# sirandreww/citizensassemblies-replication

Hardware: AMD Instinct MI355X
Metric: LEGACY panels/sec (node) at sf_e_110 shape; XtX MFMA util; speedup vs CPU (higher is better)
Workload: dtype int32/u64 (integer draw), fp4 MFMA -> exact int pairs; 1 GPU; sf_e_110: 1000000 LEGACY panels/GPU/step, k=110, n=1727, C=7, F=31, counts+pairs+unique; instance=sf_e_110, parallelism=panel shards x1, pipeline=draws on their own stream, 2 steps ahead of the counting

## Files before the change

### citizensassemblies-replication_amd/_native.py

```python
import ctypes
import os
import subprocess

HERE = os.path.dirname(os.path.abspath(__file__))
REPO = os.path.dirname(HERE)
LIB_PATH = os.environ.get("CSA_LIB") or os.path.join(HERE, "libcsa_legacy.so")
SRC = os.path.join(HERE, "csrc", "csa_legacy.hip")
SRC_MT = os.path.join(HERE, "csrc", "legacy_mt.cpp")
HEADER = os.path.join(REPO, "include", "csa_legacy.h")

CSA_OK = 0
CSA_E_INVALID = 1
CSA_E_BAD_QUOTAS = 2
CSA_E_NO_CANDIDATE = 3
CSA_E_ATTEMPT_LIMIT = 4
CSA_E_UNSUPPORTED = 5
CSA_E_HIP = 6
CSA_E_SELECTION = 7

CSA_WANT_PANELS = 0x1
CSA_WANT_COUNTS = 0x2
CSA_WANT_PAIRS = 0x4
CSA_WANT_UNIQUE = 0x8

CSA_PAIR_FP4 = 0
CSA_PAIR_I8 = 1
CSA_PAIR_OVERWRITE = 0x100
CSA_PAIR_SHARED = 0x200
CSA_PAIR_ALONE = 0x400
CSA_DRAW_RESET_STATUS = 0x1
CSA_DRAW_RESET_STATS = 0x2
CSA_PORTFOLIO_ACCUMULATE = 0x1
CSA_GROUP_WHIST_ACCUMULATE = 0x1
CSA_PRICE_ACCUMULATE = 0x1
CSA_PRICE_NONE = 0xFFFFFFFFFFFFFFFF
CSA_ADDRESS_GENERAL = 0
CSA_ADDRESS_BATCH = 1
CSA_MAXIMIN_START = 0x1
CSA_NASH_START = 0x1

_P = ctypes.c_void_p
_I32 = ctypes.c_int32
_U32 = ctypes.c_uint32
_U64 = ctypes.c_uint64
SIGNATURES = {
    "csa_version": (ctypes.c_int, []),
    "csa_last_error": (ctypes.c_char_p, []),
    "csa_device_count": (ctypes.c_int, [_P]),
    "csa_current_device": (ctypes.c_int, [_P]),
    "csa_instance_create": (ctypes.c_int, [_I32, _I32, _I32, _P, _P, _P, _P, _P]),
    "csa_instance_destroy": (None, [_P]),
    "csa_instance_info": (ctypes.c_int, [_P, _P, _P, _P, _P]),
    "csa_instance_set_state": (ctypes.c_int, [_P, _P, _P, _P]),
    "csa_legacy_sample": (ctypes.c_int, [_P, _I32, _U64, _U64, _U64, _U32, _U32, _P, _P, _P, _P, _P]),
    "csa_legacy_sample_devices": (ctypes.c_int, [_P, _P, _I32, _I32, _U64, _U64, _U64, _U32, _U32, _P, _P, _P,
                                                 _P, _P]),
    "csa_legacy_find": (ctypes.c_int, [_P, _I32, _U64, _U64, _U64, _U32, _P, _P]),
    "csa_legacy_attempt": (ctypes.c_int, [_P, _I32, _U64, _U64, _U32, _P, _P, _P, _P, _P]),
    "csa_first_panel_not_in": (ctypes.c_int, [_P, _I32, _U64, _U64, _U64, _U32, _P, _U64, _U64, _P, _P]),
    "csa_draw_round_panels": (ctypes.c_int, [_P, _I32, _P]),
    "csa_draw_async": (ctypes.c_int, [_P, _I32, _U64, _U64, _U64, _U32, _P, _P, _P, _P, _P, _P]),
    "csa_redraw_async": (ctypes.c_int, [_P, _I32, _U64, _U64, _U64, _U32, _P, _P, _P]),
    "csa_picks_stride": (_I32, [_I32]),
    "csa_draw_picks_supported": (ctypes.c_int, [_P, _I32]),
    "csa_draw_picks_async": (ctypes.c_int, [_P, _I32, _U64, _U64, _U64, _U32, _P, _P, _P, _P]),
    "csa_picks_pack_async": (ctypes.c_int, [_P, _U64, _I32, _I32, _P, _P, _P]),
    "csa_panel_hash_async": (ctypes.c_int, [_P, _U64, _I32, _P, _P]),
    "csa_draw_kernel_name": (ctypes.c_int, [_P, _I32, ctypes.c_char_p, _U64]),
    "csa_draw_kernel_list": (ctypes.c_int, [ctypes.c_char_p, _U64]),
    "csa_xt_pad": (_I32, [_I32]),
    "csa_transpose_count_async": (ctypes.c_int, [_P, _U64, _I32, _P, _P, _P]),
    "csa_pair_scratch_bytes": (_U64, [_I32, _U64, _U32]),
    "csa_pair_counts_ex_async": (ctypes.c_int, [_P, _U64, _I32, _P, _U32, _P, _U64, _P]),
    "csa_pair_counts_async": (ctypes.c_int, [_P, _U64, _I32, _P, _P]),
    "csa_unique_async": (ctypes.c_int, [_P, _P, _U64, _I32, _P, _U64, _P, _P, _P]),
    "csa_unique_mult_scratch_bytes": (_U64, [_U64]),
    "csa_unique_mult_async": (ctypes.c_int, [_P, _P, _U64, _I32, _P, _U64, _P, _P, _P, _P, _P]),
    "csa_mult_spectrum_async": (ctypes.c_int, [_P, _P, _U64, _P, _U64, _P, _P]),
    "csa_pair_histogram_async": (ctypes.c_int, [_P, _I32, _P, _U64, _P, _P]),
    "csa_unique_segments_async": (ctypes.c_int, [_P, _P, _U32, _U64, _P, _I32, _P, _U64, _P, _P, _P]),
    "csa_exchange_scratch_bytes": (_U64, [_U64]),
    "csa_exchange_pack_async": (ctypes.c_int, [_P, _P, _U64, _I32, _U32, _U64, _P, _U64, _P, _P, _P, _P, _P]),
    "csa_pairs_pack_async": (ctypes.c_int, [_P, _I32, _P, _P]),
    "csa_pairs_unpack_async": (ctypes.c_int, [_P, _I32, _P, _P]),
    "csa_pairs_upper_async": (ctypes.c_int, [_P, _I32, ctypes.c_double, _P, _P]),
    "csa_pairs_diag_async": (ctypes.c_int, [_P, _I32, _P, _P]),
    "csa_portfolio_pairs_async": (ctypes.c_int, [_P, _U64, _I32, _P, _P, _P, _U32, _P]),
    "csa_group_hist_async": (ctypes.c_int, [_P, _U64, _I32, _P, _I32, _I32, _P, _P, _P]),
    "csa_group_whist_scratch_bytes": (_U64, [_U64, _I32]),
    "csa_group_whist_scratch": (ctypes.c_int, [_P, _U64]),
    "csa_group_whist_async": (ctypes.c_int, [_P, _U64, _I32, _P, _P, _I32, _I32, _P, _U32, _P, _P]),
    "csa_draw_xt_async": (ctypes.c_int, [_P, _I32, _U64, _U64, _U64, _U32, _P, _P, _P, _P, _P, _P, _U32, _P]),
    "csa_status_decode": (ctypes.c_int, [_P]),
    "csa_legacy_draw_mt": (ctypes.c_int, [_I32, _I32, _I32, _P, _P, _P, _P, _P, _P, _P, _I32, _P, _U64, _U32,
                                          _I32, _P, _P, _P, _P, _P, _P, _P]),
    "csa_instance_set_address": (ctypes.c_int, [_P, _P]),
    "csa_instance_set_address_route": (ctypes.c_int, [_P, _I32]),
    "csa_draw_household_kernel_list": (ctypes.c_int, [ctypes.c_char_p, _U64]),
    "csa_instance_draw_stats": (ctypes.c_int, [_P, _I32, _P]),
    "csa_instance_draw_stats_reset": (ctypes.c_int, [_P, _P]),
    "csa_instance_draw_stats_async": (ctypes.c_int, [_P, _P, _P]),
    "csa_exchange_keys_async": (ctypes.c_int, [_P, _P, _U64, _I32, _U64, _U32, _U64, _P, _U64, _P, _P, _P, _P]),
    "csa_unique_keys_scratch_bytes": (_U64, [_U64, _I32]),
    "csa_unique_keys_async": (ctypes.c_int, [_P, _I32, _U64, _U32, _P, _U32, _U64, _P, _P, _U64, _P, _P, _P]),
    "csa_exchange_mult_keys_async": (ctypes.c_int, [_P, _U64, _P, _P, _P, _U64, _U32, _U64, _P, _P, _P, _P]),
    "csa_merge_mult_keys_scratch_bytes": (_U64, [_U64, _I32]),
    "csa_merge_mult_keys_async": (ctypes.c_int, [_P, _I32, _U64, _U32, _P, _U32, _U64, _P, _P, _U64, _P, _P, _P, _P,
                                                 _P]),
    "csa_rows_sort_tile": (_I32, []),
    "csa_rows_sort_scratch_bytes": (_U64, [_U64, _I32]),
    "csa_rows_sort_unique_async": (ctypes.c_int, [_P, _U64, _I32, _U64, _P, _U64, _P, _P, _P, _P, _P, _P]),
    "csa_rows_merge_scratch_bytes": (_U64, [_U64, _U64, _I32]),
    "csa_rows_merge_unique_async": (ctypes.c_int, [_P, _P, _P, _P, _U64, _P, _P, _P, _P, _U64, _I32, _P, _U64, _P, _P,
                                                   _P, _U64, _P, _P, _P]),
    "csa_rows_join_scratch_bytes": (_U64, [_U64, _U64, _I32]),
    "csa_rows_join_async": (ctypes.c_int, [_P, _P, _P, _U64, _P, _P, _P, _U64, _I32, _U32, _U64, _U64, _P, _U64, _P,
                                           _P, _P, _U64, _P, _P, _P, _P]),
    "csa_rows_find_async": (ctypes.c_int, [_P, _P, _U64, _I32, _P, _U64, _P, _P]),
    "csa_rows_price_tile": (_U64, []),
    "csa_rows_price_scratch_bytes": (_U64, [_U64, _I32]),
    "csa_rows_price_async": (ctypes.c_int, [_P, _P, _U64, _I32, _I32, _P, _U64, _U32, _P, _P, _P, _U64, _P]),
    "csa_rows_mw_cover_async": (ctypes.c_int, [_P, _P, _U64, _I32, _I32, _U32, _P, _P, _P, _P, _P, _U64, _P]),
    "csa_rows_first_holder_async": (ctypes.c_int, [_P, _P, _U64, _I32, _I32, _P, _P]),
    "csa_rows_maximin_scratch_bytes": (_U64, [_U64, _I32]),
    "csa_rows_maximin_async": (ctypes.c_int, [_P, _P, _U64, _I32, _I32, _U32, ctypes.c_double, _U32, _U32, _P, _P, _P,
# ... 94 lines not shown
```

### citizensassemblies-replication_amd/csrc/csa_legacy.hip

```cpp
#include <hip/hip_runtime.h>

#include <algorithm>
#include <type_traits>
#include <cstdlib>
#include <cstdarg>
#include <cstdio>
#include <cstring>
#include <string>
#include <vector>

#include "../../include/csa_legacy.h"

namespace {

thread_local std::string g_err;

int fail(int code, const char *fmt, ...) {
    char buf[512];
    va_list ap;
    va_start(ap, fmt);
    vsnprintf(buf, sizeof buf, fmt, ap);
    va_end(ap);
    g_err = buf;
    return code;
// ... 626 lines not shown
        }
    }
    __syncthreads();
    for (int p = threadIdx.x; p < np; p += blockDim.x)
        if (cnt[p]) atomicAdd(reinterpret_cast<unsigned long long *>(counts + p0 + p), (unsigned long long)cnt[p]);
}

typedef int v4i __attribute__((ext_vector_type(4)));
typedef int v8i __attribute__((ext_vector_type(8)));
typedef int v16i __attribute__((ext_vector_type(16)));
typedef float v16f __attribute__((ext_vector_type(16)));

constexpr int kPairBlock = 256;
constexpr int kPairThreads = 512;
constexpr int kPairKB = 8;

__device__ __forceinline__ v4i i8_frag(uint64_t w, int ks, int h) {
    const uint32_t x = (uint32_t)(w >> (32 * ks));
    v4i r;
#pragma unroll
    for (int q = 0; q < 4; ++q) r[q] = (int)((x >> (4 * h + q)) & 0x01010101u);
    return r;
}

__device__ __forceinline__ v8i f4_frag_a(uint32_t x) {
    v8i r;
    r[0] = (int)(x & 0x11111111u);
    r[1] = (int)(x & 0x22222222u);
    r[2] = (int)(x & 0x44444444u);
    r[3] = (int)((x >> 1) & 0x44444444u);
    r[4] = r[5] = r[6] = r[7] = 0;
    return r;
}
__device__ __forceinline__ v8i f4_frag_b(uint32_t x) {
    v8i r;
    r[0] = (int)((x << 2) & 0x44444444u);
    r[1] = (int)(x & 0x22222222u);
    r[2] = (int)((x >> 2) & 0x11111111u);
    r[3] = (int)((x >> 3) & 0x11111111u);
    r[4] = r[5] = r[6] = r[7] = 0;
    return r;
}

__device__ __forceinline__ void tri_block(int tri, int nbt, int &bi, int &bj) {
    bi = 0;
    int rem = tri;
    while (rem >= nbt - bi) {
        rem -= nbt - bi;
        ++bi;
    }
    bj = bi + rem;
}

template <bool FP4, bool PARTIAL, int KB>
__global__ __launch_bounds__(kPairThreads) void pair_mfma_kernel(const uint64_t *__restrict__ xt,
                                                                 uint64_t nblk, int n, int npad,
                                                                 int nbt, int nsplit,
                                                                 int64_t *__restrict__ pairs,
                                                                 int32_t *__restrict__ part) {
    __shared__ uint64_t words[2][KB][2 * kPairBlock];
    const int t = threadIdx.x, lane = t & 63, wave = t >> 6;
    const int g = (int)blockIdx.x, G = (int)gridDim.x, ntri = nbt * (nbt + 1) / 2;
    const int xcd = g & 7, it = xcd * (G >> 3) + min(xcd, G & 7) + (g >> 3);
    const int split = it / ntri, tri = it - split * ntri;
    const int item = tri * nsplit + split;
    int bi, bj;
    tri_block(tri, nbt, bi, bj);
    const int I0 = bi * kPairBlock, J0 = bj * kPairBlock;
    const uint64_t per = (nblk + nsplit - 1) / nsplit;
    const uint64_t kb0 = min(nblk, (uint64_t)split * per), kb1 = min(nblk, kb0 + per);

    using acc_t = typename std::conditional<FP4, v16f, v16i>::type;
    acc_t acc[4][2];
#pragma unroll
    for (int a = 0; a < 4; ++a)
#pragma unroll
        for (int b = 0; b < 2; ++b)
#pragma unroll
            for (int v = 0; v < 16; ++v) acc[a][b][v] = 0;

    const int wr = wave >> 2, wc = wave & 3;
    const int r32 = lane & 31, h = lane >> 5;
    const int src = t < kPairBlock ? I0 + t : J0 + t - kPairBlock;
    uint64_t nw[KB];
    const uint64_t nst = (kb1 - kb0 + KB - 1) / KB;
    auto load_stage = [&](uint64_t s) {
#pragma unroll
        for (int j = 0; j < KB; ++j) {
            const uint64_t b = kb0 + s * KB + j;
            const uint32_t *x32 = reinterpret_cast<const uint32_t *>(xt) + 2 * b * (uint64_t)npad + src;
            nw[j] = b < kb1 ? ((uint64_t)x32[0] | ((uint64_t)x32[npad] << 32)) : 0ull;
        }
    };
    if (nst) {
        load_stage(0);
#pragma unroll
        for (int j = 0; j < KB; ++j) words[0][j][t] = nw[j];
        if (nst > 1) load_stage(1);
    }
    __syncthreads();
    for (uint64_t s = 0; s < nst; ++s) {
        const int buf = (int)(s & 1);
#pragma unroll
        for (int j = 0; j < KB; ++j) {
            {
                const uint64_t *w = words[buf][j];
                if constexpr (FP4) {
                    const uint32_t *w32 = reinterpret_cast<const uint32_t *>(w) + h;
                    v8i fa[4], fb[2];
#pragma unroll
                    for (int x = 0; x < 4; ++x) fa[x] = f4_frag_a(w32[2 * (128 * wr + 32 * x + r32)]);
#pragma unroll
                    for (int x = 0; x < 2; ++x) fb[x] = f4_frag_b(w32[2 * (kPairBlock + 64 * wc + 32 * x + r32)]);
#pragma unroll
                    for (int a = 0; a < 4; ++a)
#pragma unroll
                        for (int b = 0; b < 2; ++b)
                            acc[a][b] = __builtin_amdgcn_mfma_scale_f32_32x32x64_f8f6f4(
                                fa[a], fb[b], acc[a][b], 4, 4, 0, 0x7F7F7F7F, 0, 0x7F7F7F7F);
                } else {
                    uint64_t wa[4], wb[2];
#pragma unroll
                    for (int x = 0; x < 4; ++x) wa[x] = w[128 * wr + 32 * x + r32];
#pragma unroll
                    for (int x = 0; x < 2; ++x) wb[x] = w[kPairBlock + 64 * wc + 32 * x + r32];
#pragma unroll
                    for (int ks = 0; ks < 2; ++ks) {
                        v4i fa[4], fb[2];
#pragma unroll
                        for (int x = 0; x < 4; ++x) fa[x] = i8_frag(wa[x], ks, h);
#pragma unroll
                        for (int x = 0; x < 2; ++x) fb[x] = i8_frag(wb[x], ks, h);
#pragma unroll
                        for (int a = 0; a < 4; ++a)
#pragma unroll
                            for (int b = 0; b < 2; ++b)
                                acc[a][b] = __builtin_amdgcn_mfma_i32_32x32x32_i8(fa[a], fb[b], acc[a][b], 0, 0, 0);
                    }
                }
            }
            if (j == 0) {
                if (s + 1 < nst) {
#pragma unroll
                    for (int jj = 0; jj < KB; ++jj) words[buf ^ 1][jj][t] = nw[jj];
                }
                if (s + 2 < nst) load_stage(s + 2);
            }
        }
        __syncthreads();
    }
    const int rloc = 128 * wr + 4 * h, cloc = 64 * wc + r32;
    if constexpr (PARTIAL) {
        int32_t *dst = part + (size_t)item * kPairBlock * kPairBlock;
#pragma unroll
        for (int a = 0; a < 4; ++a)
#pragma unroll
            for (int b = 0; b < 2; ++b)
#pragma unroll
                for (int v = 0; v < 16; ++v) {
                    const int row = rloc + 32 * a + (v & 3) + 8 * (v >> 2);
                    dst[row * kPairBlock + cloc + 32 * b] = (int)acc[a][b][v];
                }
    } else {
#pragma unroll
        for (int a = 0; a < 4; ++a)
#pragma unroll
            for (int b = 0; b < 2; ++b) {
                const int col = J0 + cloc + 32 * b;
#pragma unroll
                for (int v = 0; v < 16; ++v) {
                    const int row = I0 + rloc + 32 * a + (v & 3) + 8 * (v >> 2);
                    const int val = (int)acc[a][b][v];
                    if (val != 0 && row < n && col < n)
                        atomicAdd(reinterpret_cast<unsigned long long *>(pairs + (uint64_t)row * n + col),
                                  (unsigned long long)(long long)val);
                }
                __builtin_amdgcn_sched_barrier(0);
            }
    }
}

__global__ __launch_bounds__(256) void pair_reduce_kernel(const int32_t *__restrict__ part, int n, int nbt,
                                                          int nsplit, int64_t *__restrict__ pairs,
                                                          int overwrite) {
    int bi, bj;
    tri_block((int)blockIdx.y, nbt, bi, bj);
    const int e = blockIdx.x * 256 + threadIdx.x;
    const int row = bi * kPairBlock + (e >> 8), col = bj * kPairBlock + (e & 255);
    if (row >= n || col >= n) return;
    const int32_t *p = part + (size_t)blockIdx.y * nsplit * kPairBlock * kPairBlock + e;
    int64_t acc = 0;
    for (int k = 0; k < nsplit; ++k) acc += p[(size_t)k * kPairBlock * kPairBlock];
    if (overwrite) pairs[(size_t)row * n + col] = acc;
    else if (acc) pairs[(size_t)row * n + col] += acc;
}

constexpr int kP2Threads = 256;
constexpr int kP2Depth = 8;
constexpr int kP2Xcds = 8;
constexpr uint64_t kP2MaxBlocks = ((1ull << 24) - 1) / 64;

struct PairMap {
    int nbt, ntri, P;
    int halves;
    uint64_t nblk;
    __host__ __device__ int nitems() const { return ntri * halves; }
    __host__ __device__ void item_at(int idx, int &bi, int &bj, int &c0) const {
        tile_at(idx / halves, bi, bj);
        c0 = (idx % halves) * (kPairBlock / halves);
    }
    __host__ __device__ void tile_at(int idx, int &bi, int &bj) const {
        int r0 = 0;
        for (;;) {
            const int hb = nbt - r0 < 4 ? nbt - r0 : 4;
            const int cnt = hb * (hb + 1) / 2 + (nbt - r0 - hb) * hb;
            if (idx < cnt) break;
            idx -= cnt;
            r0 += 4;
        }
        const int hb = nbt - r0 < 4 ? nbt - r0 : 4;
        const int tri = hb * (hb + 1) / 2;
        if (idx < tri) {
            int c = 0;
            while (idx > c) {
                idx -= c + 1;
                ++c;
            }
            bj = r0 + c;
            bi = r0 + idx;
        } else {
            idx -= tri;
            bj = r0 + hb + idx / hb;
            bi = r0 + idx % hb;
        }
    }
    __host__ __device__ void xcd_chunk(int x, int &t0, int &tx) const {
        t0 = (int)((int64_t)nitems() * x / kP2Xcds);
        tx = (int)((int64_t)nitems() * (x + 1) / kP2Xcds) - t0;
    }
    __host__ __device__ int leftovers() const {
        int tl = 0;
        for (int x = 0; x < kP2Xcds; ++x) {
            int t0, tx;
// ... 1540 lines not shown
    for (const DrawConfig &c : kDrawKernels) {
        draw_config_name(c, name, sizeof name);
        all += name;
        all += '\n';
    }
    if (!buf || len < all.size() + 1)
        return fail(CSA_E_INVALID, "draw kernel list: the buffer needs %zu bytes", all.size() + 1);
    memcpy(buf, all.c_str(), all.size() + 1);
    return CSA_OK;
}

int csa_draw_household_kernel_list(char *buf, uint64_t len) {
    std::string all;
    char name[128];
    for (const DrawConfig &c : kHouseholdKernels) {
        draw_config_name(c, name, sizeof name);
        all += name;
        all += '\n';
    }
    if (!buf || len < all.size() + 1)
        return fail(CSA_E_INVALID, "household kernel list: the buffer needs %zu bytes", all.size() + 1);
    memcpy(buf, all.c_str(), all.size() + 1);
    return CSA_OK;
}

int32_t csa_xt_pad(int32_t n) { return ((n + kPairBlock - 1) / kPairBlock) * kPairBlock; }

int csa_transpose_count_async(const uint64_t *d_panels, uint64_t n_panels, int32_t n, uint64_t *d_xt,
                              int64_t *d_counts, void *stream) {
    if (n <= 0 || !d_panels || !d_counts) return fail(CSA_E_INVALID, "transpose: bad arguments");
    if (n_panels == 0) return CSA_OK;
    const int W = (n + 63) / 64, CW = std::min(W, kXtCols), Wp = CW | 1;
    const size_t lds = (size_t)64 * Wp * 8 + (size_t)std::min(n, 64 * CW) * 4;
    if (lds > 160 * 1024) return fail(CSA_E_UNSUPPORTED, "transpose needs %zu B of LDS", lds);
    const uint64_t nblk = (n_panels + 63) / 64;
    const unsigned ranges = (unsigned)((W + kXtCols - 1) / kXtCols);
    static int cus = 0;
    if (!cus) {
        int dev = 0;
        if (hipGetDevice(&dev) != hipSuccess ||
            hipDeviceGetAttribute(&cus, hipDeviceAttributeMultiprocessorCount, dev) != hipSuccess || cus <= 0)
            cus = 256;
    }
    const uint64_t bpg = std::max<uint64_t>(1, std::min<uint64_t>(kXtBlocksPerGroup, nblk * ranges / (2 * (uint64_t)cus)));
    const unsigned grid = (unsigned)((nblk + bpg - 1) / bpg);
    hipLaunchKernelGGL(xt_count_kernel, dim3(grid, ranges), dim3(kXtThreads), lds, (hipStream_t)stream, d_panels,
                       n_panels, n, W, csa_xt_pad(n), d_xt, d_counts, (int)bpg);
    HIPCHK(hipGetLastError());
    return CSA_OK;
}

namespace {
struct PairPlan {
    int npad, nbt, ntri, nsplit;
};

int pair_plan(int32_t n, uint64_t n_blocks, uint32_t engine, PairPlan &p) {
    if (engine != CSA_PAIR_FP4 && engine != CSA_PAIR_I8) return fail(CSA_E_INVALID, "pairs: unknown engine %u", engine);
    p.npad = csa_xt_pad(n);
    p.nbt = p.npad / kPairBlock;
    p.ntri = p.nbt * (p.nbt + 1) / 2;
    int cus = 256;
    int dev = 0;
    if (hipGetDevice(&dev) == hipSuccess) (void)hipDeviceGetAttribute(&cus, hipDeviceAttributeMultiprocessorCount, dev);
    const uint64_t ns_cap = std::max<uint64_t>(1, n_blocks / 8);
    uint64_t ns = std::max(1, cus / p.ntri);
    if (2 * p.ntri > cus) {
        auto cost = [&](uint64_t m) { return (double)((p.ntri * m + cus - 1) / cus) / (double)m; };
        const uint64_t hi = std::min<uint64_t>(64, ns_cap);
        double best = cost(1);
        for (uint64_t m = 2; m <= hi; ++m) best = std::min(best, cost(m));
        ns = 1;
        while (ns < hi && cost(ns) > 1.02 * best) ++ns;
    }
    ns = std::min<uint64_t>(ns, ns_cap);
    const uint64_t exact_blocks = engine == CSA_PAIR_FP4 ? (1ull << 24) / 64 : (1ull << 31) / 64;
    ns = std::max<uint64_t>(ns, (n_blocks + exact_blocks - 1) / exact_blocks);
    if (ns > (1u << 20)) return fail(CSA_E_UNSUPPORTED, "pairs: too many panel blocks per call");
    p.nsplit = (int)ns;
    return CSA_OK;
}
struct Pair2Plan {
    PairMap M;
    int grid = 0, lmax = 0;
};

constexpr uint64_t kP2AloneMinBlocks = 2048;
constexpr int kP2AloneMinTiles = 4;
bool pair2_plan(int32_t n, uint64_t n_blocks, uint32_t engine, bool shared, Pair2Plan &q, bool alone = false) {
    if (engine != CSA_PAIR_FP4 || n_blocks == 0 || n_blocks > kP2MaxBlocks) return false;
    const char *e = getenv("CSA_PAIR_KERNEL");
    const int force = e ? atoi(e) : 0;
    if (force == 1) return false;
    int cus = 256, dev = 0;
    if (hipGetDevice(&dev) == hipSuccess) (void)hipDeviceGetAttribute(&cus, hipDeviceAttributeMultiprocessorCount, dev);
    if (cus < kP2Xcds || cus % kP2Xcds) return false;
    (void)shared;
    const char *enb = getenv("CSA_P2_NB");
    const int nbf = enb ? atoi(enb) : 4;
    q.M.halves = nbf == 2 ? 2 : 1;
    q.M.nbt = csa_xt_pad(n) / kPairBlock;
    q.M.ntri = q.M.nbt * (q.M.nbt + 1) / 2;
    q.M.P = cus / kP2Xcds;
    q.M.nblk = n_blocks;
    q.grid = cus;
    q.lmax = q.M.leftovers();
    static const uint64_t alone_min_blocks = [] {
        const char *v = getenv("CSA_PAIR_ALONE_MIN_BLOCKS");
        return v ? (uint64_t)strtoull(v, nullptr, 10) : kP2AloneMinBlocks;
    }();
    alone = alone && n_blocks >= alone_min_blocks && q.M.nbt >= kP2AloneMinTiles;
    return force == 2 || alone || q.M.ntri >= cus;
}

uint64_t pair2_scratch_bytes(const Pair2Plan &q) {
    return q.lmax ? (uint64_t)q.lmax * q.M.pieces(q.lmax) * kPairBlock * kPairBlock * sizeof(int32_t) : 0;
}
}

uint64_t csa_pair_scratch_bytes(int32_t n, uint64_t n_blocks, uint32_t engine) {
    engine &= ~(CSA_PAIR_OVERWRITE | CSA_PAIR_SHARED | CSA_PAIR_ALONE);
    if (n <= 0 || n_blocks == 0) return 0;
    uint64_t need = 0;
    Pair2Plan q;
    if (pair2_plan(n, n_blocks, engine, false, q, true)) need = std::max<uint64_t>(pair2_scratch_bytes(q), 4);
    if (pair2_plan(n, n_blocks, engine, false, q)) return need;
    PairPlan p;
    if (pair_plan(n, n_blocks, engine, p)) return need;
    return std::max<uint64_t>(need, (uint64_t)p.ntri * p.nsplit * kPairBlock * kPairBlock * sizeof(int32_t));
}

int csa_pair_counts_ex_async(const uint64_t *d_xt, uint64_t n_blocks, int32_t n, int64_t *d_pairs,
                             uint32_t engine, void *d_scratch, uint64_t scratch_bytes, void *stream) {
    if (n <= 0 || !d_xt || !d_pairs) return fail(CSA_E_INVALID, "pairs: bad arguments");
    const bool overwrite = (engine & CSA_PAIR_OVERWRITE) != 0u, shared = (engine & CSA_PAIR_SHARED) != 0u;
    const bool alone = (engine & CSA_PAIR_ALONE) != 0u && !shared;
    engine &= ~(CSA_PAIR_OVERWRITE | CSA_PAIR_SHARED | CSA_PAIR_ALONE);
    const hipStream_t st = (hipStream_t)stream;
    if (overwrite && (n_blocks == 0 || !d_scratch))
        HIPCHK(hipMemsetAsync(d_pairs, 0, (size_t)n * n * sizeof(int64_t), st));
    if (n_blocks == 0) return CSA_OK;
    Pair2Plan q;
    if (d_scratch && pair2_plan(n, n_blocks, engine, shared, q, alone)) {
        if (scratch_bytes < pair2_scratch_bytes(q))
            return fail(CSA_E_INVALID, "pairs: scratch of %llu B < csa_pair_scratch_bytes = %llu B",
                        (unsigned long long)scratch_bytes, (unsigned long long)pair2_scratch_bytes(q));
        int32_t *part = static_cast<int32_t *>(d_scratch);
        const uint32_t *xt32 = reinterpret_cast<const uint32_t *>(d_xt);
        const int npad = csa_xt_pad(n), ow = overwrite ? 1 : 0;
        const void *fn = q.M.halves == 2 ? reinterpret_cast<const void *>(&pair_fp4_tile_kernel<2>)
                                         : reinterpret_cast<const void *>(&pair_fp4_tile_kernel<4>);
        PairMap M = q.M;
        void *args[] = {(void *)&xt32, &n, (void *)&npad, &M, &d_pairs, &part, (void *)&ow};
        HIPCHK(hipLaunchKernel(fn, dim3(q.grid), dim3(kP2Threads), args, 0, st));
        HIPCHK(hipGetLastError());
        if (q.lmax) {
            hipLaunchKernelGGL(pair_reduce2_kernel, dim3(kPairBlock, q.lmax), dim3(kPairBlock), 0, st,
                               (const int32_t *)part, n, q.M, d_pairs, ow);
            HIPCHK(hipGetLastError());
        }
        return CSA_OK;
    }
    PairPlan p;
    int rc = pair_plan(n, n_blocks, engine, p);
    if (rc) return rc;
    const bool partial = d_scratch != nullptr;
    if (partial && scratch_bytes < csa_pair_scratch_bytes(n, n_blocks, engine))
        return fail(CSA_E_INVALID, "pairs: scratch of %llu B < csa_pair_scratch_bytes = %llu B",
                    (unsigned long long)scratch_bytes, (unsigned long long)csa_pair_scratch_bytes(n, n_blocks, engine));
    const dim3 grid(p.ntri * p.nsplit), block(kPairThreads);
    int32_t *part = static_cast<int32_t *>(d_scratch);
    const void *fn = engine == CSA_PAIR_FP4
                         ? (partial ? reinterpret_cast<const void *>(&pair_mfma_kernel<true, true, kPairKB>)
                                    : reinterpret_cast<const void *>(&pair_mfma_kernel<true, false, kPairKB>))
                         : (partial ? reinterpret_cast<const void *>(&pair_mfma_kernel<false, true, kPairKB>)
                                    : reinterpret_cast<const void *>(&pair_mfma_kernel<false, false, kPairKB>));
    uint64_t nb = n_blocks;
    int npad = p.npad, nbt = p.nbt, nsplit = p.nsplit;
    void *args[] = {(void *)&d_xt, &nb, &n, &npad, &nbt, &nsplit, &d_pairs, &part};
    HIPCHK(hipLaunchKernel(fn, grid, block, args, 0, st));
    HIPCHK(hipGetLastError());
    if (partial) {
        hipLaunchKernelGGL(pair_reduce_kernel, dim3(kPairBlock, p.ntri), dim3(256), 0, st, part, n, p.nbt, p.nsplit,
                           d_pairs, (int)overwrite);
        HIPCHK(hipGetLastError());
    }
    return CSA_OK;
}

int csa_pair_counts_async(const uint64_t *d_xt, uint64_t n_blocks, int32_t n, int64_t *d_pairs, void *stream) {
    return csa_pair_counts_ex_async(d_xt, n_blocks, n, d_pairs, CSA_PAIR_FP4, nullptr, 0, stream);
}

int csa_unique_async(const uint64_t *d_hashes, const uint64_t *d_panels, uint64_t n_panels, int32_t W,
                     uint64_t *d_table, uint64_t table_slots, uint64_t *d_unique, uint32_t *d_status, void *stream) {
    return unique_impl(d_hashes, d_panels, n_panels, W, d_table, table_slots, d_unique, d_status, 0, nullptr,
                       (hipStream_t)stream);
}

int csa_unique_segments_async(const uint64_t *d_hashes, const uint64_t *d_panels, uint32_t n_segments,
                              uint64_t capacity, const uint64_t *d_seg_counts, int32_t W, uint64_t *d_table,
                              uint64_t table_slots, uint64_t *d_unique, uint32_t *d_status, void *stream) {
    if (!d_seg_counts || capacity == 0 || capacity > 0xFFFFFFFFull)
        return fail(CSA_E_INVALID, "unique segments: bad arguments");
    return unique_impl(d_hashes, d_panels, (uint64_t)n_segments * capacity, W, d_table, table_slots, d_unique,
                       d_status, (uint32_t)capacity, d_seg_counts, (hipStream_t)stream);
}

static uint64_t mult_global_slots(uint64_t n) { return pow2_at_least(std::max<uint64_t>(2 * n, 64)); }

uint64_t csa_unique_mult_scratch_bytes(uint64_t n_panels) {
    const uint64_t n = std::max<uint64_t>(n_panels, 1);
    UqPlan q;
    uq_plan(n, q);
    return std::max<uint64_t>(q.scratch_bytes, 12 * mult_global_slots(n));
}

int csa_unique_mult_async(const uint64_t *d_hashes, const uint64_t *d_panels, uint64_t n_panels, int32_t W,
                          void *d_scratch, uint64_t scratch_bytes, uint32_t *d_first, uint32_t *d_mult,
                          uint64_t *d_distinct, uint32_t *d_status, void *stream) {
    if (W < 1 || !d_distinct) return fail(CSA_E_INVALID, "unique mult: bad arguments");
    if (n_panels && (!d_hashes || !d_panels || !d_scratch || !d_first || !d_mult))
        return fail(CSA_E_INVALID, "unique mult: NULL pointer with %llu panels", (unsigned long long)n_panels);
    if (n_panels >= (1ull << 32)) return fail(CSA_E_UNSUPPORTED, "unique mult: n_panels >= 2^32 (u32 indices)");
    if (n_panels && scratch_bytes < csa_unique_mult_scratch_bytes(n_panels))
        return fail(CSA_E_INVALID, "unique mult: scratch_bytes < csa_unique_mult_scratch_bytes(n_panels)");
    const hipStream_t st = (hipStream_t)stream;
    unsigned long long *len = reinterpret_cast<unsigned long long *>(d_distinct);
    HIPCHK(hipMemsetAsync(len, 0, 8, st));
    if (n_panels == 0) return CSA_OK;
    UqPlan q;
    uq_plan(n_panels, q);
    const char *ue = getenv("CSA_UNIQUE_PART");
    if (d_status && n_panels >= 65536 && q.fits && q.scratch_bytes <= scratch_bytes && !(ue && atoi(ue) == 0)) {
        uint32_t *idx = static_cast<uint32_t *>(d_scratch);
        uint32_t *pbase = uq_partition(d_hashes, n_panels, q, idx, 0, nullptr, st);
        hipLaunchKernelGGL(uq_mult_kernel, dim3((unsigned)q.P), dim3(kUqThreads), 0, st, d_hashes, d_panels, W, idx,
// ... 1181 lines not shown
```

### include/csa_legacy.h

```cpp
#ifndef CSA_LEGACY_H
#define CSA_LEGACY_H

#include <stddef.h>
#include <stdint.h>

#ifdef __cplusplus
extern "C" {
#endif

#define CSA_OK 0
#define CSA_E_INVALID 1
#define CSA_E_BAD_QUOTAS 2
#define CSA_E_NO_CANDIDATE 3
#define CSA_E_ATTEMPT_LIMIT 4
#define CSA_E_UNSUPPORTED 5
#define CSA_E_HIP 6
#define CSA_E_SELECTION 7

#define CSA_WANT_PANELS 0x1u
#define CSA_WANT_COUNTS 0x2u
#define CSA_WANT_PAIRS 0x4u
#define CSA_WANT_UNIQUE 0x8u

typedef struct csa_instance csa_instance;
// ... 45 lines not shown
                           uint64_t m, uint64_t chunk, int64_t *index_out, uint64_t *panel_out);

int csa_legacy_draw_mt(int32_t n, int32_t C, int32_t F, const int32_t *person_feat, const int32_t *fmin,
                       const int32_t *fmax, const int32_t *sel0, const int32_t *rem0, const uint64_t *present0,
                       const int32_t *addr_next, int32_t k, uint32_t *mt_state, uint64_t n_panels,
                       uint32_t max_attempts, int32_t single, int32_t *picks_out, uint64_t *panels_out,
                       uint32_t *attempts_out, int32_t *sel_out, int32_t *rem_out, uint64_t *present_out,
                       uint64_t *stats_out);


int csa_draw_round_panels(const csa_instance *inst, int32_t k, uint64_t *out);

int csa_draw_async(const csa_instance *inst, int32_t k, uint64_t seed, uint64_t panel_begin,
                   uint64_t n_panels, uint32_t max_attempts, uint64_t *d_panels,
                   uint64_t *d_hashes, uint32_t *d_attempts, int32_t *d_picks,
                   uint32_t *d_status, void *stream);
#define CSA_DRAW_RESET_STATUS 0x1u
#define CSA_DRAW_RESET_STATS 0x2u
int csa_draw_xt_async(const csa_instance *inst, int32_t k, uint64_t seed, uint64_t panel_begin,
                      uint64_t n_panels, uint32_t max_attempts, uint64_t *d_panels, uint64_t *d_hashes,
                      uint32_t *d_attempts, uint32_t *d_status, uint32_t *d_xt, int32_t *xt_written,
                      uint32_t flags, void *stream);

int csa_redraw_async(const csa_instance *inst, int32_t k, uint64_t seed, uint64_t panel_begin,
                     uint64_t n_panels, uint32_t max_attempts, uint64_t *d_panels, uint32_t *d_status,
                     void *stream);

int32_t csa_picks_stride(int32_t k);
int csa_draw_picks_supported(const csa_instance *inst, int32_t k);
int csa_draw_picks_async(const csa_instance *inst, int32_t k, uint64_t seed, uint64_t panel_begin,
                         uint64_t n_panels, uint32_t max_attempts, uint16_t *d_picks, uint32_t *d_attempts,
                         uint32_t *d_status, void *stream);
int csa_picks_pack_async(const uint16_t *d_picks, uint64_t n_panels, int32_t k, int32_t n, uint64_t *d_panels,
                         uint64_t *d_hashes, void *stream);

int csa_panel_hash_async(const uint64_t *d_panels, uint64_t n_panels, int32_t W, uint64_t *d_hashes,
                         void *stream);

int csa_draw_kernel_name(const csa_instance *inst, int32_t k, char *buf, uint64_t len);

int csa_draw_kernel_list(char *buf, uint64_t len);
int csa_draw_household_kernel_list(char *buf, uint64_t len);

int32_t csa_xt_pad(int32_t n);
int csa_transpose_count_async(const uint64_t *d_panels, uint64_t n_panels, int32_t n,
                              uint64_t *d_xt, int64_t *d_counts, void *stream);

#define CSA_PAIR_FP4 0u
#define CSA_PAIR_I8 1u
#define CSA_PAIR_OVERWRITE 0x100u
#define CSA_PAIR_SHARED 0x200u
#define CSA_PAIR_ALONE 0x400u
uint64_t csa_pair_scratch_bytes(int32_t n, uint64_t n_blocks, uint32_t engine);
int csa_pair_counts_ex_async(const uint64_t *d_xt, uint64_t n_blocks, int32_t n, int64_t *d_pairs,
                             uint32_t engine, void *d_scratch, uint64_t scratch_bytes, void *stream);
int csa_pair_counts_async(const uint64_t *d_xt, uint64_t n_blocks, int32_t n, int64_t *d_pairs,
                          void *stream);

int csa_unique_async(const uint64_t *d_hashes, const uint64_t *d_panels, uint64_t n_panels, int32_t W,
                     uint64_t *d_table, uint64_t table_slots, uint64_t *d_unique, uint32_t *d_status,
                     void *stream);

int csa_pair_histogram_async(const int64_t *d_pairs, int32_t n, uint64_t *d_hist, uint64_t n_bins,
                             uint64_t *d_overflow, void *stream);

int csa_unique_segments_async(const uint64_t *d_hashes, const uint64_t *d_panels, uint32_t n_segments,
                              uint64_t capacity, const uint64_t *d_seg_counts, int32_t W, uint64_t *d_table,
                              uint64_t table_slots, uint64_t *d_unique, uint32_t *d_status, void *stream);

uint64_t csa_unique_mult_scratch_bytes(uint64_t n_panels);
int csa_unique_mult_async(const uint64_t *d_hashes, const uint64_t *d_panels, uint64_t n_panels, int32_t W,
                          void *d_scratch, uint64_t scratch_bytes, uint32_t *d_first, uint32_t *d_mult,
                          uint64_t *d_distinct, uint32_t *d_status, void *stream);

int csa_mult_spectrum_async(const uint32_t *d_mult, const uint64_t *d_distinct, uint64_t capacity,
                            uint64_t *d_spectrum, uint64_t n_bins, uint64_t *d_summary, void *stream);

uint64_t csa_exchange_scratch_bytes(uint64_t n_panels);
int csa_exchange_pack_async(const uint64_t *d_hashes, const uint64_t *d_panels, uint64_t n_panels, int32_t W,
                            uint32_t world, uint64_t capacity, void *d_scratch, uint64_t scratch_bytes,
                            uint64_t *d_send_hashes, uint64_t *d_send_panels, uint64_t *d_send_counts,
                            uint32_t *d_status, void *stream);

int csa_exchange_keys_async(const uint64_t *d_hashes, const uint64_t *d_panels, uint64_t n_panels, int32_t W,
                            uint64_t panel_begin, uint32_t world, uint64_t capacity, void *d_scratch,
                            uint64_t scratch_bytes, uint64_t *d_send_keys, uint64_t *d_send_counts,
                            uint32_t *d_status, void *stream);
uint64_t csa_unique_keys_scratch_bytes(uint64_t n_keys, int32_t W);
int csa_unique_keys_async(const csa_instance *inst, int32_t k, uint64_t seed, uint32_t max_attempts,
                          const uint64_t *d_keys, uint32_t n_segments, uint64_t capacity,
                          const uint64_t *d_seg_counts, void *d_scratch, uint64_t scratch_bytes,
                          uint64_t *d_unique, uint32_t *d_status, void *stream);

int csa_exchange_mult_keys_async(const uint64_t *d_hashes, uint64_t n_panels, const uint32_t *d_first,
                                 const uint32_t *d_mult, const uint64_t *d_distinct, uint64_t panel_begin,
                                 uint32_t world, uint64_t capacity, uint64_t *d_send_keys,
                                 uint64_t *d_send_counts, uint32_t *d_status, void *stream);
uint64_t csa_merge_mult_keys_scratch_bytes(uint64_t n_keys, int32_t W);
int csa_merge_mult_keys_async(const csa_instance *inst, int32_t k, uint64_t seed, uint32_t max_attempts,
                              const uint64_t *d_keys, uint32_t n_segments, uint64_t capacity,
                              const uint64_t *d_seg_counts, void *d_scratch, uint64_t scratch_bytes,
                              uint32_t *d_first, uint32_t *d_mult, uint64_t *d_distinct, uint32_t *d_status,
                              void *stream);

int32_t csa_rows_sort_tile(void);
uint64_t csa_rows_sort_scratch_bytes(uint64_t n_rows, int32_t W);
// ... 87 lines not shown
```

Baseline: 298.2 million panels/s.

## Skip masked MFMA tiles on diagonal blocks and split diagonal work separately

The pair-count MFMA kernel now skips 32x32 sub-tiles that lie below the diagonal or beyond n, using a per-wave mask, and keeps a full unmasked path for interior off-diagonal blocks. Diagonal blocks get remapped wave assignments and their own K-split count, chosen by a cost model, so the grid can give lighter diagonal tiles a different split than off-diagonal ones. The goal is to cut wasted MFMA work on triangle and edge tiles and to balance the load across CUs. In exchange, indexing gets more complex, the masked path adds branches, and a new plan API and env override are added.

New measurement: 293.5 million panels/s. -1.6%, worse.

```diff
diff --git a/citizensassemblies-replication_amd/_native.py b/citizensassemblies-replication_amd/_native.py
--- a/citizensassemblies-replication_amd/_native.py
+++ b/citizensassemblies-replication_amd/_native.py
@@ -71,6 +71,8 @@
     "csa_xt_pad": (_I32, [_I32]),
     "csa_transpose_count_async": (ctypes.c_int, [_P, _U64, _I32, _P, _P, _P]),
     "csa_pair_scratch_bytes": (_U64, [_I32, _U64, _U32]),
+    "csa_pair_plan": (ctypes.c_int, [_I32, _U64, _U32, _P, _P, _P]),
+    "csa_pair_piece_begin": (_U64, [_U64, _I32, _I32]),
     "csa_pair_counts_ex_async": (ctypes.c_int, [_P, _U64, _I32, _P, _U32, _P, _U64, _P]),
     "csa_pair_counts_async": (ctypes.c_int, [_P, _U64, _I32, _P, _P]),
     "csa_unique_async": (ctypes.c_int, [_P, _P, _U64, _I32, _P, _U64, _P, _P, _P]),
diff --git a/citizensassemblies-replication_amd/csrc/csa_legacy.hip b/citizensassemblies-replication_amd/csrc/csa_legacy.hip
--- a/citizensassemblies-replication_amd/csrc/csa_legacy.hip
+++ b/citizensassemblies-replication_amd/csrc/csa_legacy.hip
@@ -702,23 +702,136 @@
     bj = bi + rem;
 }
 
+struct PairSplits {
+    int nbt, ord, diag;
+    __host__ __device__ int pieces(int bi, int bj) const { return bi == bj ? diag : ord; }
+    __host__ __device__ int slot0(int tri, int bi, int bj) const { return tri * ord + (bi + (bj > bi)) * (diag - ord); }
+    __host__ __device__ int items() const { return nbt * diag + (nbt * (nbt + 1) / 2 - nbt) * ord; }
+};
+__host__ __device__ inline uint64_t pair_cut(uint64_t nblk, int ns, int s) { return nblk * (uint64_t)s / (uint64_t)ns; }
+
+__device__ __forceinline__ uint32_t pair_wave_mask(int bi, int bj, int n, int wr, int wc) {
+    uint32_t m = 0;
+#pragma unroll
+    for (int a = 0; a < 4; ++a)
+#pragma unroll
+        for (int b = 0; b < 2; ++b) {
+            const int R = 4 * wr + a, C = 2 * wc + b;
+            if (bi * kPairBlock + 32 * R < n && bj * kPairBlock + 32 * C < n && (bi < bj || R <= C)) m |= 1u << (2 * a + b);
+        }
+    return m;
+}
+
+template <bool FP4, bool MASKED, typename acc_t>
+__device__ __forceinline__ void pair_word(const uint64_t *w, int wr, int wc, int r32, int h, uint32_t mask,
+                                          acc_t (&acc)[4][2]) {
+    if constexpr (FP4) {
+        const uint32_t *w32 = reinterpret_cast<const uint32_t *>(w) + h;
+        if constexpr (!MASKED) {
+            v8i fa[4], fb[2];
+#pragma unroll
+            for (int x = 0; x < 4; ++x) fa[x] = f4_frag_a(w32[2 * (128 * wr + 32 * x + r32)]);
+#pragma unroll
+            for (int x = 0; x < 2; ++x) fb[x] = f4_frag_b(w32[2 * (kPairBlock + 64 * wc + 32 * x + r32)]);
+#pragma unroll
+            for (int a = 0; a < 4; ++a)
+#pragma unroll
+                for (int b = 0; b < 2; ++b)
+                    acc[a][b] = __builtin_amdgcn_mfma_scale_f32_32x32x64_f8f6f4(
+                        fa[a], fb[b], acc[a][b], 4, 4, 0, 0x7F7F7F7F, 0, 0x7F7F7F7F);
+        } else if (mask) {
+            v8i fb[2];
+#pragma unroll
+            for (int x = 0; x < 2; ++x) fb[x] = f4_frag_b(w32[2 * (kPairBlock + 64 * wc + 32 * x + r32)]);
+#pragma unroll
+            for (int a = 0; a < 4; ++a) {
+                if ((mask >> (2 * a)) & 3u) {
+                    const v8i fa = f4_frag_a(w32[2 * (128 * wr + 32 * a + r32)]);
+#pragma unroll
+                    for (int b = 0; b < 2; ++b)
+                        if ((mask >> (2 * a + b)) & 1u)
+                            acc[a][b] = __builtin_amdgcn_mfma_scale_f32_32x32x64_f8f6f4(
+                                fa, fb[b], acc[a][b], 4, 4, 0, 0x7F7F7F7F, 0, 0x7F7F7F7F);
+                }
+            }
+        }
+    } else {
+        if constexpr (!MASKED) {
+            uint64_t wa[4], wb[2];
+#pragma unroll
+            for (int x = 0; x < 4; ++x) wa[x] = w[128 * wr + 32 * x + r32];
+#pragma unroll
+            for (int x = 0; x < 2; ++x) wb[x] = w[kPairBlock + 64 * wc + 32 * x + r32];
+#pragma unroll
+            for (int ks = 0; ks < 2; ++ks) {
+                v4i fa[4], fb[2];
+#pragma unroll
+                for (int x = 0; x < 4; ++x) fa[x] = i8_frag(wa[x], ks, h);
+#pragma unroll
+                for (int x = 0; x < 2; ++x) fb[x] = i8_frag(wb[x], ks, h);
+#pragma unroll
+                for (int a = 0; a < 4; ++a)
+#pragma unroll
+                    for (int b = 0; b < 2; ++b)
+                        acc[a][b] = __builtin_amdgcn_mfma_i32_32x32x32_i8(fa[a], fb[b], acc[a][b], 0, 0, 0);
+            }
+        } else if (mask) {
+#pragma unroll
+            for (int ks = 0; ks < 2; ++ks) {
+                v4i fb[2];
+#pragma unroll
+                for (int x = 0; x < 2; ++x) fb[x] = i8_frag(w[kPairBlock + 64 * wc + 32 * x + r32], ks, h);
+#pragma unroll
+                for (int a = 0; a < 4; ++a) {
+                    if ((mask >> (2 * a)) & 3u) {
+                        const v4i fa = i8_frag(w[128 * wr + 32 * a + r32], ks, h);
+#pragma unroll
+                        for (int b = 0; b < 2; ++b)
+                            if ((mask >> (2 * a + b)) & 1u)
+                                acc[a][b] = __builtin_amdgcn_mfma_i32_32x32x32_i8(fa, fb[b], acc[a][b], 0, 0, 0);
+                    }
+                }
+            }
+        }
+    }
+}
+
 template <bool FP4, bool PARTIAL, int KB>
 __global__ __launch_bounds__(kPairThreads) void pair_mfma_kernel(const uint64_t *__restrict__ xt,
                                                                  uint64_t nblk, int n, int npad,
-                                                                 int nbt, int nsplit,
+                                                                 PairSplits P,
                                                                  int64_t *__restrict__ pairs,
                                                                  int32_t *__restrict__ part) {
     __shared__ uint64_t words[2][KB][2 * kPairBlock];
-    const int t = threadIdx.x, lane = t & 63, wave = t >> 6;
+    const int t = threadIdx.x, lane = t & 63, wave = __builtin_amdgcn_readfirstlane(t >> 6);
+    const int nbt = P.nbt;
     const int g = (int)blockIdx.x, G = (int)gridDim.x, ntri = nbt * (nbt + 1) / 2;
     const int xcd = g & 7, it = xcd * (G >> 3) + min(xcd, G & 7) + (g >> 3);
-    const int split = it / ntri, tri = it - split * ntri;
-    const int item = tri * nsplit + split;
+    const int smin = min(P.ord, P.diag);
+    int split, tri;
+    if (it < smin * ntri) {
+        split = it / ntri;
+        tri = it - split * ntri;
+    } else {
+        const bool dmore = P.diag > P.ord;
+        const int nc = dmore ? nbt : ntri - nbt, r = it - smin * ntri;
+        split = smin + r / nc;
+        int k = r - (split - smin) * nc, row = k;
+        if (!dmore) {
+            row = 0;
+            while (k >= nbt - 1 - row) {
+                k -= nbt - 1 - row;
+                ++row;
+            }
+        }
+        tri = row * nbt - row * (row - 1) / 2 + (dmore ? 0 : 1 + k);
+    }
     int bi, bj;
     tri_block(tri, nbt, bi, bj);
+    const int item = P.slot0(tri, bi, bj) + split;
     const int I0 = bi * kPairBlock, J0 = bj * kPairBlock;
-    const uint64_t per = (nblk + nsplit - 1) / nsplit;
-    const uint64_t kb0 = min(nblk, (uint64_t)split * per), kb1 = min(nblk, kb0 + per);
+    const int nsp = P.pieces(bi, bj);
+    const uint64_t kb0 = pair_cut(nblk, nsp, split), kb1 = pair_cut(nblk, nsp, split + 1);
 
     using acc_t = typename std::conditional<FP4, v16f, v16i>::type;
     acc_t acc[4][2];
@@ -729,7 +842,10 @@
 #pragma unroll
             for (int v = 0; v < 16; ++v) acc[a][b][v] = 0;
 
-    const int wr = wave >> 2, wc = wave & 3;
+    const int wsel = bi == bj ? (int)((0x60547132u >> (4 * wave)) & 15u) : wave;
+    const int wr = wsel >> 2, wc = wsel & 3;
+    const bool full = FP4 && bi < bj && J0 + kPairBlock <= n;
+    const uint32_t mask = __builtin_amdgcn_readfirstlane(pair_wave_mask(bi, bj, n, wr, wc));
     const int r32 = lane & 31, h = lane >> 5;
     const int src = t < kPairBlock ? I0 + t : J0 + t - kPairBlock;
     uint64_t nw[KB];
@@ -749,56 +865,25 @@
         if (nst > 1) load_stage(1);
     }
     __syncthreads();
-    for (uint64_t s = 0; s < nst; ++s) {
-        const int buf = (int)(s & 1);
-#pragma unroll
-        for (int j = 0; j < KB; ++j) {
-            {
-                const uint64_t *w = words[buf][j];
-                if constexpr (FP4) {
-                    const uint32_t *w32 = reinterpret_cast<const uint32_t *>(w) + h;
-                    v8i fa[4], fb[2];
-#pragma unroll
-                    for (int x = 0; x < 4; ++x) fa[x] = f4_frag_a(w32[2 * (128 * wr + 32 * x + r32)]);
-#pragma unroll
-                    for (int x = 0; x < 2; ++x) fb[x] = f4_frag_b(w32[2 * (kPairBlock + 64 * wc + 32 * x + r32)]);
-#pragma unroll
-                    for (int a = 0; a < 4; ++a)
-#pragma unroll
-                        for (int b = 0; b < 2; ++b)
-                            acc[a][b] = __builtin_amdgcn_mfma_scale_f32_32x32x64_f8f6f4(
-                                fa[a], fb[b], acc[a][b], 4, 4, 0, 0x7F7F7F7F, 0, 0x7F7F7F7F);
-                } else {
-                    uint64_t wa[4], wb[2];
-#pragma unroll
-                    for (int x = 0; x < 4; ++x) wa[x] = w[128 * wr + 32 * x + r32];
-#pragma unroll
-                    for (int x = 0; x < 2; ++x) wb[x] = w[kPairBlock + 64 * wc + 32 * x + r32];
-#pragma unroll
-                    for (int ks = 0; ks < 2; ++ks) {
-                        v4i fa[4], fb[2];
-#pragma unroll
-                        for (int x = 0; x < 4; ++x) fa[x] = i8_frag(wa[x], ks, h);
-#pragma unroll
-                        for (int x = 0; x < 2; ++x) fb[x] = i8_frag(wb[x], ks, h);
-#pragma unroll
-                        for (int a = 0; a < 4; ++a)
-#pragma unroll
-                            for (int b = 0; b < 2; ++b)
-                                acc[a][b] = __builtin_amdgcn_mfma_i32_32x32x32_i8(fa[a], fb[b], acc[a][b], 0, 0, 0);
+    auto run = [&](auto masked) {
+        for (uint64_t s = 0; s < nst; ++s) {
+            const int buf = (int)(s & 1);
+#pragma unroll
+            for (int j = 0; j < KB; ++j) {
+                pair_word<FP4, decltype(masked)::value>(words[buf][j], wr, wc, r32, h, mask, acc);
+                if (j == 0) {
+                    if (s + 1 < nst) {
+#pragma unroll
+                        for (int jj = 0; jj < KB; ++jj) words[buf ^ 1][jj][t] = nw[jj];
                     }
+                    if (s + 2 < nst) load_stage(s + 2);
                 }
             }
-            if (j == 0) {
-                if (s + 1 < nst) {
-#pragma unroll
-                    for (int jj = 0; jj < KB; ++jj) words[buf ^ 1][jj][t] = nw[jj];
-                }
-                if (s + 2 < nst) load_stage(s + 2);
-            }
-        }
-        __syncthreads();
-    }
+            __syncthreads();
+        }
+    };
+    if (full) run(std::false_type{});
+    else run(std::true_type{});
     const int rloc = 128 * wr + 4 * h, cloc = 64 * wc + r32;
     if constexpr (PARTIAL) {
         int32_t *dst = part + (size_t)item * kPairBlock * kPairBlock;
@@ -830,15 +915,15 @@
     }
 }
 
-__global__ __launch_bounds__(256) void pair_reduce_kernel(const int32_t *__restrict__ part, int n, int nbt,
-                                                          int nsplit, int64_t *__restrict__ pairs,
-                                                          int overwrite) {
+__global__ __launch_bounds__(256) void pair_reduce_kernel(const int32_t *__restrict__ part, int n, PairSplits P,
+                                                          int64_t *__restrict__ pairs, int overwrite) {
     int bi, bj;
-    tri_block((int)blockIdx.y, nbt, bi, bj);
+    tri_block((int)blockIdx.y, P.nbt, bi, bj);
     const int e = blockIdx.x * 256 + threadIdx.x;
     const int row = bi * kPairBlock + (e >> 8), col = bj * kPairBlock + (e & 255);
     if (row >= n || col >= n) return;
-    const int32_t *p = part + (size_t)blockIdx.y * nsplit * kPairBlock * kPairBlock + e;
+    const int nsplit = P.pieces(bi, bj);
+    const int32_t *p = part + (size_t)P.slot0((int)blockIdx.y, bi, bj) * kPairBlock * kPairBlock + e;
     int64_t acc = 0;
     for (int k = 0; k < nsplit; ++k) acc += p[(size_t)k * kPairBlock * kPairBlock];
     if (overwrite) pairs[(size_t)row * n + col] = acc;
@@ -2485,8 +2570,13 @@
 
 namespace {
 struct PairPlan {
-    int npad, nbt, ntri, nsplit;
+    int npad, nbt, ntri;
+    int ord, diag;
+    PairSplits splits() const { return PairSplits{nbt, ord, diag}; }
+    uint64_t slots() const { return (uint64_t)splits().items(); }
 };
+
+constexpr double kPairDiagCost = 0.625;
 
 int pair_plan(int32_t n, uint64_t n_blocks, uint32_t engine, PairPlan &p) {
     if (engine != CSA_PAIR_FP4 && engine != CSA_PAIR_I8) return fail(CSA_E_INVALID, "pairs: unknown engine %u", engine);
@@ -2507,10 +2597,30 @@
         while (ns < hi && cost(ns) > 1.02 * best) ++ns;
     }
     ns = std::min<uint64_t>(ns, ns_cap);
-    const uint64_t exact_blocks = engine == CSA_PAIR_FP4 ? (1ull << 24) / 64 : (1ull << 31) / 64;
-    ns = std::max<uint64_t>(ns, (n_blocks + exact_blocks - 1) / exact_blocks);
-    if (ns > (1u << 20)) return fail(CSA_E_UNSUPPORTED, "pairs: too many panel blocks per call");
-    p.nsplit = (int)ns;
+    uint64_t ord = ns, diag = ns;
+    const uint64_t nd = (uint64_t)p.nbt, no = (uint64_t)(p.ntri - p.nbt);
+    if (2 * p.ntri <= cus && no) {
+        double best = std::max(1.0, kPairDiagCost) / (double)ns;
+        for (uint64_t a = 1; a <= ns_cap && no * a + nd <= (uint64_t)cus; ++a) {
+            const uint64_t b = std::min<uint64_t>(ns_cap, ((uint64_t)cus - no * a) / nd);
+            const double t = std::max(1.0 / (double)a, kPairDiagCost / (double)b);
+            if (t < best * (1.0 - 1e-9)) best = t, ord = a, diag = b;
+        }
+    }
+    if (const char *e = getenv("CSA_PAIR_SPLITS")) {
+        unsigned a = 0, b = 0;
+        if (sscanf(e, "%u,%u", &a, &b) == 2 && a && b) {
+            ord = std::min<uint64_t>(a, ns_cap);
+            diag = no ? std::min<uint64_t>(b, ns_cap) : ord;
+        }
+    }
+    const uint64_t exact_blocks = engine == CSA_PAIR_FP4 ? ((1ull << 24) - 1) / 64 : ((1ull << 31) - 1) / 64;
+    const uint64_t ns_exact = (n_blocks + exact_blocks - 1) / exact_blocks;
+    ord = std::max(ord, ns_exact);
+    diag = std::max(diag, ns_exact);
+    if (ord > (1u << 20) || diag > (1u << 20)) return fail(CSA_E_UNSUPPORTED, "pairs: too many panel blocks per call");
+    p.ord = (int)ord;
+    p.diag = (int)diag;
     return CSA_OK;
 }
 struct Pair2Plan {
@@ -2560,7 +2670,26 @@
     if (pair2_plan(n, n_blocks, engine, false, q)) return need;
     PairPlan p;
     if (pair_plan(n, n_blocks, engine, p)) return need;
-    return std::max<uint64_t>(need, (uint64_t)p.ntri * p.nsplit * kPairBlock * kPairBlock * sizeof(int32_t));
+    return std::max<uint64_t>(need, p.slots() * kPairBlock * kPairBlock * sizeof(int32_t));
+}
+
+int csa_pair_plan(int32_t n, uint64_t n_blocks, uint32_t engine, int32_t *out3, uint64_t *items, uint64_t *slots) {
+    engine &= ~(CSA_PAIR_OVERWRITE | CSA_PAIR_SHARED | CSA_PAIR_ALONE);
+    if (n <= 0 || n_blocks == 0 || !out3) return fail(CSA_E_INVALID, "pair plan: bad arguments");
+    PairPlan p;
+    int rc = pair_plan(n, n_blocks, engine, p);
+    if (rc) return rc;
+    out3[0] = p.nbt;
+    out3[1] = p.ord;
+    out3[2] = p.diag;
+    if (items) *items = (uint64_t)p.splits().items();
+    if (slots) *slots = p.slots();
+    return CSA_OK;
+}
+
+uint64_t csa_pair_piece_begin(uint64_t n_blocks, int32_t pieces, int32_t piece) {
+    if (pieces <= 0 || piece <= 0) return 0;
+    return piece >= pieces ? n_blocks : pair_cut(n_blocks, pieces, piece);
 }
 
 int csa_pair_counts_ex_async(const uint64_t *d_xt, uint64_t n_blocks, int32_t n, int64_t *d_pairs,
@@ -2601,7 +2730,7 @@
     if (partial && scratch_bytes < csa_pair_scratch_bytes(n, n_blocks, engine))
         return fail(CSA_E_INVALID, "pairs: scratch of %llu B < csa_pair_scratch_bytes = %llu B",
                     (unsigned long long)scratch_bytes, (unsigned long long)csa_pair_scratch_bytes(n, n_blocks, engine));
-    const dim3 grid(p.ntri * p.nsplit), block(kPairThreads);
+    const dim3 grid((unsigned)p.splits().items()), block(kPairThreads);
     int32_t *part = static_cast<int32_t *>(d_scratch);
     const void *fn = engine == CSA_PAIR_FP4
                          ? (partial ? reinterpret_cast<const void *>(&pair_mfma_kernel<true, true, kPairKB>)
@@ -2609,13 +2738,14 @@
                          : (partial ? reinterpret_cast<const void *>(&pair_mfma_kernel<false, true, kPairKB>)
                                     : reinterpret_cast<const void *>(&pair_mfma_kernel<false, false, kPairKB>));
     uint64_t nb = n_blocks;
-    int npad = p.npad, nbt = p.nbt, nsplit = p.nsplit;
-    void *args[] = {(void *)&d_xt, &nb, &n, &npad, &nbt, &nsplit, &d_pairs, &part};
+    int npad = p.npad;
+    PairSplits sp = p.splits();
+    void *args[] = {(void *)&d_xt, &nb, &n, &npad, &sp, &d_pairs, &part};
     HIPCHK(hipLaunchKernel(fn, grid, block, args, 0, st));
     HIPCHK(hipGetLastError());
     if (partial) {
-        hipLaunchKernelGGL(pair_reduce_kernel, dim3(kPairBlock, p.ntri), dim3(256), 0, st, part, n, p.nbt, p.nsplit,
-                           d_pairs, (int)overwrite);
+        hipLaunchKernelGGL(pair_reduce_kernel, dim3(kPairBlock, p.ntri), dim3(256), 0, st, part, n, sp, d_pairs,
+                           (int)overwrite);
         HIPCHK(hipGetLastError());
     }
     return CSA_OK;
diff --git a/include/csa_legacy.h b/include/csa_legacy.h
--- a/include/csa_legacy.h
+++ b/include/csa_legacy.h
@@ -121,6 +121,9 @@
 #define CSA_PAIR_SHARED 0x200u
 #define CSA_PAIR_ALONE 0x400u
 uint64_t csa_pair_scratch_bytes(int32_t n, uint64_t n_blocks, uint32_t engine);
+int csa_pair_plan(int32_t n, uint64_t n_blocks, uint32_t engine, int32_t *out3, uint64_t *items,
+                  uint64_t *slots);
+uint64_t csa_pair_piece_begin(uint64_t n_blocks, int32_t pieces, int32_t piece);
 int csa_pair_counts_ex_async(const uint64_t *d_xt, uint64_t n_blocks, int32_t n, int64_t *d_pairs,
                              uint32_t engine, void *d_scratch, uint64_t scratch_bytes, void *stream);
 int csa_pair_counts_async(const uint64_t *d_xt, uint64_t n_blocks, int32_t n, int64_t *d_pairs,
```
